# One-2-3-45/One-2-3-45

Hardware: NVIDIA H100
Metric: sec/mesh end-to-end (256x256 in) (lower is better)
Workload: dtype f16

## Files before the change

### one-2-3-45_b200/csrc/gemm_tc.cu

```cuda
#include <cuda.h>
#include <stdlib.h>
#include <cuda_fp16.h>

#include "common.cuh"
#include "wgmma.cuh"

namespace o2345 {
namespace {

constexpr int BM = 128, BK = 64;
constexpr int EPI_WARPS = 8;
constexpr int EPI_THREADS = 32 * EPI_WARPS;
constexpr int GEMM_THREADS = 128 + EPI_THREADS;
constexpr uint64_t WAIT_LIMIT_NS = 4000000000ull;
constexpr int MAX_CLUSTER = 8;
constexpr int RES_PREFETCH = 8;

enum { WAIT_EMPTY = 1, WAIT_FULL = 2 };

struct TrapRecord {
  unsigned long long magic;
  int tag, stage, bx, by, bz, rank, M, N, K, bn, mode, splits, conv;
};
constexpr unsigned long long TRAP_MAGIC = 0x6f32333435545250ull;

__device__ __forceinline__ uint32_t smem_u32(const void* p) { return (uint32_t)__cvta_generic_to_shared(p); }

__device__ __forceinline__ void mbar_init(uint64_t* bar, uint32_t count) {
  asm volatile("mbarrier.init.shared::cta.b64 [%0], %1;" ::"r"(smem_u32(bar)), "r"(count));
}
__device__ __forceinline__ void mbar_expect_tx(uint64_t* bar, uint32_t bytes) {
  asm volatile("mbarrier.arrive.expect_tx.shared::cta.b64 _, [%0], %1;" ::"r"(smem_u32(bar)), "r"(bytes) : "memory");
}
__device__ __forceinline__ void mbar_arrive(uint64_t* bar) {
  asm volatile("mbarrier.arrive.shared::cta.b64 _, [%0];" ::"r"(smem_u32(bar)) : "memory");
}
__device__ __forceinline__ uint32_t mbar_try(uint64_t* bar, uint32_t parity) {
  uint32_t done;
  asm volatile(
      "{\n\t.reg .pred p;\n\t"
      "mbarrier.try_wait.parity.shared::cta.b64 p, [%1], %2;\n\t"
      "selp.u32 %0, 1, 0, p;\n\t}"
      : "=r"(done)
      : "r"(smem_u32(bar)), "r"(parity)
      : "memory");
  return done;
}
__device__ __forceinline__ uint64_t global_ns() {
  uint64_t t;
  asm volatile("mov.u64 %0, %%globaltimer;" : "=l"(t));
  return t;
}
__device__ __forceinline__ void tma_load_2d(void* dst, const CUtensorMap* map, uint64_t* bar, int c0, int c1) {
  asm volatile(
      "cp.async.bulk.tensor.2d.shared::cluster.global.mbarrier::complete_tx::bytes [%0], [%1, {%3, %4}], [%2];"
      ::"r"(smem_u32(dst)), "l"(map), "r"(smem_u32(bar)), "r"(c0), "r"(c1)
      : "memory");
}
__device__ __forceinline__ void tma_load_4d(void* dst, const CUtensorMap* map, uint64_t* bar, int c0, int c1, int c2, int c3) {
  asm volatile(
      "cp.async.bulk.tensor.4d.shared::cluster.global.mbarrier::complete_tx::bytes [%0], [%1, {%3, %4, %5, %6}], [%2];"
      ::"r"(smem_u32(dst)), "l"(map), "r"(smem_u32(bar)), "r"(c0), "r"(c1), "r"(c2), "r"(c3)
      : "memory");
}
__device__ __forceinline__ uint32_t cluster_ctarank() {
  uint32_t r;
  asm volatile("mov.u32 %0, %%cluster_ctarank;" : "=r"(r));
  return r;
}
__device__ __forceinline__ void cluster_sync_all() {
  asm volatile("barrier.cluster.arrive.release.aligned;\n\tbarrier.cluster.wait.acquire.aligned;" ::: "memory");
}
__device__ __forceinline__ void epi_bar() { asm volatile("bar.sync 1, 256;" ::: "memory"); }

__host__ __device__ constexpr int acc_ld(int bn) { return bn + 4; }
__device__ __forceinline__ void acc_ld32(const float* src, uint32_t (&r)[32]) {
#pragma unroll
  for (int i = 0; i < 8; ++i) {
    const float4 v = reinterpret_cast<const float4*>(src)[i];
    r[4 * i] = __float_as_uint(v.x), r[4 * i + 1] = __float_as_uint(v.y), r[4 * i + 2] = __float_as_uint(v.z), r[4 * i + 3] = __float_as_uint(v.w);
  }
}

struct GemmParams {
  int M, N, K;
  int64_t ldc;
  int nh;
  int64_t stride_c_h, stride_c_b;
  const float* bias;
  const __half* rowbias;
  int64_t rowbias_ld;
  int rows_per_group;
  const __half* residual;
  void* C;
  int out_f32;
  int act;
// ... 211 lines not shown
  }
  const int share = (BM * BN + p.splits - 1) / p.splits;
  const int i1 = min(BM * BN, (z + 1) * share);
  for (int i = z * share + te; i < i1; i += EPI_THREADS) {
    const int rl = i / BN, row = m0 + rl, col = n0 + (i - rl * BN);
    if (row >= p.M || col >= p.N) continue;
    float x = 0.f;
    for (int s = 0; s < p.splits; ++s) x += __ldcg(p.ws + (int64_t)s * plane + (int64_t)row * p.N + col);
    x *= p.alpha;
    if (p.rowbias) x += __half2float(p.rowbias[(int64_t)(row / p.rows_per_group) * p.rowbias_ld + col]);
    if (p.bias) x += __ldg(p.bias + col);
    x = apply_act(x, p.act);
    const int64_t o = out_row(p, row) * p.ldc + col;
    if (p.residual) x += __half2float(p.residual[o]);
    if (p.out_f32) reinterpret_cast<float*>(p.C)[o] = x;
    else reinterpret_cast<__half*>(p.C)[o] = __float2half_rn(x);
  }
}

constexpr int EPI_RB_GROUPS = 8;
__host__ __device__ constexpr int epi_smem_bytes(int bn) { return bn * 4 + EPI_RB_GROUPS * bn * 2; }
__host__ __device__ constexpr int col_split(int bn) { return ((bn / 2 + 31) / 32) * 32; }

template <int BN>
__device__ __forceinline__ void epilogue_preload(const GemmParams& p, int m0, int n0, float* sbias, __half* srb, int te) {
  for (int i = te; i < BN; i += EPI_THREADS) sbias[i] = (p.bias && n0 + i < p.N) ? __ldg(p.bias + n0 + i) : 0.f;
  if (p.rowbias) {
    const int g0 = m0 / p.rows_per_group;
    const int last = (m0 + BM - 1 < p.M ? m0 + BM - 1 : p.M - 1) / p.rows_per_group;
    const int ng = last - g0 + 1;
    if (ng >= 1 && ng <= EPI_RB_GROUPS)
      for (int i = te; i < ng * BN; i += EPI_THREADS) {
        const int gi = i / BN, c = i - gi * BN;
        srb[i] = (n0 + c < p.N) ? p.rowbias[(int64_t)(g0 + gi) * p.rowbias_ld + n0 + c] : __float2half(0.f);
      }
  }
  epi_bar();
}

template <int ACT>
__device__ __forceinline__ float act_fn(float x) {
  if (ACT == 1) return __fdividef(x, 1.f + __expf(-x));
  if (ACT == 2) return gelu_erf(x);
  if (ACT == 4) return __fdividef(x, 1.f + __expf(-1.702f * x));
  return x;
}

template <int ACT>
__device__ __forceinline__ void stage_rows(const GemmParams& p, const float* acc_row, uint8_t* mine, int n0, int c_lo, int c_hi,
                                           const float* sbias, const __half* rb, bool rb_smem) {
#pragma unroll 1
  for (int c0 = c_lo; c0 < c_hi; c0 += 32) {
    if (n0 + c0 >= p.N) break;
    uint32_t r[32];
    acc_ld32(acc_row + c0, r);
    if (ACT == 3) {
      __half2 h[8];
#pragma unroll
      for (int e = 0; e < 16; e += 2) {
        float a0 = fmaf(__uint_as_float(r[e]), p.alpha, sbias[c0 + e]), a1 = fmaf(__uint_as_float(r[e + 1]), p.alpha, sbias[c0 + e + 1]);
        float g0 = fmaf(__uint_as_float(r[16 + e]), p.alpha, sbias[c0 + 16 + e]);
        float g1 = fmaf(__uint_as_float(r[17 + e]), p.alpha, sbias[c0 + 17 + e]);
        h[e >> 1] = __floats2half2_rn(a0 * gelu_erf_fast(g0), a1 * gelu_erf_fast(g1));
      }
      uint4* d = reinterpret_cast<uint4*>(mine + (c0 - c_lo));
      d[0] = reinterpret_cast<uint4*>(h)[0], d[1] = reinterpret_cast<uint4*>(h)[1];
    } else {
#pragma unroll
      for (int j = 0; j < 32; j += 8) {
        float v[8];
        const float4 b0 = *reinterpret_cast<const float4*>(sbias + c0 + j), b1 = *reinterpret_cast<const float4*>(sbias + c0 + j + 4);
        v[0] = b0.x, v[1] = b0.y, v[2] = b0.z, v[3] = b0.w, v[4] = b1.x, v[5] = b1.y, v[6] = b1.z, v[7] = b1.w;
        if (rb && (rb_smem || n0 + c0 + j + 8 <= p.N)) {
          uint4 q = *reinterpret_cast<const uint4*>(rb + c0 + j);
          const __half* hq = reinterpret_cast<const __half*>(&q);
#pragma unroll
          for (int e = 0; e < 8; ++e) v[e] += __half2float(hq[e]);
        }
        __half2 h[4];
#pragma unroll
        for (int e = 0; e < 8; e += 2) {
          float x0 = fmaf(__uint_as_float(r[j + e]), p.alpha, v[e]), x1 = fmaf(__uint_as_float(r[j + e + 1]), p.alpha, v[e + 1]);
          h[e >> 1] = __floats2half2_rn(act_fn<ACT>(x0), act_fn<ACT>(x1));
        }
        *reinterpret_cast<uint4*>(mine + (c0 - c_lo + j) * 2) = *reinterpret_cast<uint4*>(h);
      }
    }
  }
}

struct WarpOut {
  int outc, stride, ppr, total, ocol0, nout;
};
template <int MODE>
__device__ __forceinline__ WarpOut warp_out(const GemmParams& p, int n0, int c_lo, int c_hi) {
  constexpr bool geglu = MODE == 1;
  WarpOut g;
  g.outc = geglu ? (c_hi - c_lo) >> 1 : (c_hi - c_lo);
  g.stride = g.outc * 2 + 16;
  g.ppr = g.outc >> 3;
  g.total = 32 * g.ppr;
  g.ocol0 = geglu ? (n0 + c_lo) >> 1 : n0 + c_lo;
  g.nout = geglu ? p.N >> 1 : p.N;
  return g;
}

__device__ __forceinline__ void prefetch_residual(const GemmParams& p, const WarpOut& g, int lane, int row0,
                                                  uint4 (&resq)[RES_PREFETCH]) {
#pragma unroll
  for (int u = 0; u < RES_PREFETCH; ++u) {
    resq[u] = make_uint4(0u, 0u, 0u, 0u);
    const int pp = lane + 32 * u;
    if (p.residual && pp < g.total) {
      const int rl = pp / g.ppr, ci = pp - rl * g.ppr;
      const int grow = row0 + rl, col = g.ocol0 + ci * 8;
      if (grow < p.M && col < g.nout) resq[u] = *reinterpret_cast<const uint4*>(p.residual + out_row(p, grow) * p.ldc + col);
    }
  }
}

__device__ __forceinline__ uint4 add_h8(uint4 v, uint4 q) {
  __half2* a = reinterpret_cast<__half2*>(&v);
  const __half2* b = reinterpret_cast<const __half2*>(&q);
#pragma unroll
  for (int e = 0; e < 4; ++e) {
    float2 fa = __half22float2(a[e]), fb = __half22float2(b[e]);
    a[e] = __floats2half2_rn(fa.x + fb.x, fa.y + fb.y);
  }
  return v;
}

template <int BN, int MODE>
__device__ __forceinline__ void epilogue_staged(const GemmParams& p, const WarpOut& g, const float* acc_row, uint8_t* slab, int lane,
                                                int m0, int row0, int n0, int c_lo, int c_hi, const float* sbias, const __half* srb,
                                                const uint4 (&resq)[RES_PREFETCH]) {
  const int row = row0 + lane;
  const __half* rb = nullptr;
  bool rb_smem = false;
  if (MODE != 1 && p.rowbias) {
    const int rr = row < p.M ? row : p.M - 1;
    const int g0 = m0 / p.rows_per_group, last = (m0 + BM - 1 < p.M ? m0 + BM - 1 : p.M - 1) / p.rows_per_group;
    rb_smem = last - g0 + 1 <= EPI_RB_GROUPS;
    rb = rb_smem ? srb + (rr / p.rows_per_group - g0) * BN : p.rowbias + (int64_t)(rr / p.rows_per_group) * p.rowbias_ld + n0;
  }
  uint8_t* mine = slab + lane * g.stride;
  if (MODE == 0) {
    stage_rows<0>(p, acc_row, mine, n0, c_lo, c_hi, sbias, rb, rb_smem);
  } else if (MODE == 1) {
    stage_rows<3>(p, acc_row, mine, n0, c_lo, c_hi, sbias, rb, rb_smem);
  } else {
    switch (p.act) {
      case 1: stage_rows<1>(p, acc_row, mine, n0, c_lo, c_hi, sbias, rb, rb_smem); break;
      case 2: stage_rows<2>(p, acc_row, mine, n0, c_lo, c_hi, sbias, rb, rb_smem); break;
      default: stage_rows<4>(p, acc_row, mine, n0, c_lo, c_hi, sbias, rb, rb_smem); break;
    }
  }
  __syncwarp();
  __half* C = reinterpret_cast<__half*>(p.C);
#pragma unroll
  for (int u = 0; u < RES_PREFETCH; ++u) {
    const int pp = lane + 32 * u;
    if (pp < g.total) {
      const int rl = pp / g.ppr, ci = pp - rl * g.ppr;
      const int grow = row0 + rl, col = g.ocol0 + ci * 8;
      if (grow < p.M && col < g.nout) {
        uint4 v = *reinterpret_cast<const uint4*>(slab + rl * g.stride + ci * 16);
        if (p.residual) v = add_h8(v, resq[u]);
        *reinterpret_cast<uint4*>(C + out_row(p, grow) * p.ldc + col) = v;
      }
    }
  }
  constexpr int UN = 4;
  for (int base = lane + 32 * RES_PREFETCH; base < g.total; base += 32 * UN) {
    uint4 v[UN], q[UN];
    int64_t o[UN];
    bool ok[UN];
#pragma unroll
    for (int u = 0; u < UN; ++u) {
      const int pp = base + 32 * u;
      const int rl = pp / g.ppr, ci = pp - rl * g.ppr;
      const int grow = row0 + rl, col = g.ocol0 + ci * 8;
      ok[u] = pp < g.total && grow < p.M && col < g.nout;
      o[u] = out_row(p, grow) * p.ldc + col;
      if (ok[u]) {
        v[u] = *reinterpret_cast<const uint4*>(slab + rl * g.stride + ci * 16);
        if (p.residual) q[u] = *reinterpret_cast<const uint4*>(p.residual + o[u]);
      }
    }
#pragma unroll
    for (int u = 0; u < UN; ++u) {
      if (!ok[u]) continue;
      if (p.residual) v[u] = add_h8(v[u], q[u]);
      *reinterpret_cast<uint4*>(C + o[u]) = v[u];
    }
  }
}

__host__ __device__ constexpr int epi_slab_bytes(int bn) { return EPI_WARPS * 32 * (col_split(bn) * 2 + 16); }
constexpr int smem_bytes(int bn, int stages) {
  return stages * (BM * BK * 2 + bn * BK * 2) + epi_slab_bytes(bn) + 2 * stages * 8 + 16 + epi_smem_bytes(bn) + 1024;
}

struct ProducerPos {
  int x, y, b;
  int tap, tx, ty;
  int cb;
};
__device__ __forceinline__ ProducerPos producer_start(const GemmParams& p, int m0, int bz, int kb0) {
  ProducerPos q;
  q.x = q.y = q.b = q.tap = q.tx = q.ty = q.cb = 0;
  if (p.conv) {
    const int r = m0 / p.cW;
    q.x = m0 - r * p.cW, q.y = r % p.cH, q.b = r / p.cH;
    q.tap = kb0 / p.cblocks, q.cb = kb0 - q.tap * p.cblocks;
    q.ty = q.tap / p.ctx, q.tx = q.tap - q.ty * p.ctx;
  } else if (p.batched) {
    q.y = bz % p.nh, q.b = bz / p.nh;
  }
  return q;
}
__device__ __forceinline__ void producer_step(const GemmParams& p, ProducerPos& q) {
  if (p.conv && ++q.cb == p.cblocks) {
    q.cb = 0, ++q.tap;
// ... 10 lines not shown
    tma_load_4d(a_dst, tmA, full_bar, c0, q.x + q.tx + p.cox, q.y + q.ty + p.coy, q.b);
    tma_load_2d(b_dst, tmB, full_bar, q.tap * p.cC + c0, n0);
  } else if (p.batched) {
    tma_load_4d(a_dst, tmA, full_bar, kb * BK, m0, q.y, q.b);
    tma_load_4d(b_dst, tmB, full_bar, kb * BK, n0, q.y, q.b);
  } else {
    tma_load_2d(a_dst, tmA, full_bar, kb * BK, m0);
    tma_load_2d(b_dst, tmB, full_bar, kb * BK, n0);
  }
}

template <int BN>
__device__ __forceinline__ void acc_store(float* acc, const float (&d)[BN / 2], int row0, int t) {
  const int r = row0 + 16 * (t >> 5) + ((t & 31) >> 2), c = 2 * (t & 3);
#pragma unroll
  for (int j = 0; j < BN / 8; ++j) {
    *reinterpret_cast<float2*>(acc + r * acc_ld(BN) + 8 * j + c) = make_float2(d[4 * j], d[4 * j + 1]);
    *reinterpret_cast<float2*>(acc + (r + 8) * acc_ld(BN) + 8 * j + c) = make_float2(d[4 * j + 2], d[4 * j + 3]);
  }
}

template <int BN, int STAGES, int MODE>
__global__ void __launch_bounds__(GEMM_THREADS, 1)
gemm_tc_kernel(const __grid_constant__ CUtensorMap tmA, const __grid_constant__ CUtensorMap tmB, const __grid_constant__ GemmParams p) {
  extern __shared__ __align__(1024) uint8_t smem_raw[];
  uint8_t* smem = reinterpret_cast<uint8_t*>((reinterpret_cast<uintptr_t>(smem_raw) + 1023) & ~(uintptr_t)1023);
  constexpr int A_BYTES = BM * BK * 2, B_BYTES = BN * BK * 2;
  static_assert(B_BYTES % 1024 == 0, "stage bases must stay 1024-byte aligned for SWIZZLE_128B");
  static_assert(BN % 32 == 0 && BN >= 64 && BN <= 256, "tile width: a multiple of 32 (GEGLU chunks, 32-column epilogue reads)");
  static_assert(BM * acc_ld(BN) * 4 <= STAGES * (A_BYTES + B_BYTES), "the accumulator tile must fit in the operand ring");
  constexpr int CSPLIT = col_split(BN);
  uint8_t* sA = smem;
  uint8_t* sB = smem + STAGES * A_BYTES;
  uint8_t* slabs = sB + STAGES * B_BYTES;
  uint64_t* full = reinterpret_cast<uint64_t*>(slabs + epi_slab_bytes(BN));
  uint64_t* empty = full + STAGES;
  float* sbias = reinterpret_cast<float*>((reinterpret_cast<uintptr_t>(empty + STAGES) + 15) & ~(uintptr_t)15);
  __half* srb = reinterpret_cast<__half*>(sbias + BN);
  float* acc = reinterpret_cast<float*>(smem);

  const int warp = threadIdx.x >> 5, lane = threadIdx.x & 31;
  if (threadIdx.x == 0) stamp(p, 0), stamp_ns(p, 16);
  const int bz = blockIdx.z;
  const int nk = p.conv ? p.ctaps * p.cblocks : (p.K + BK - 1) / BK;
  const bool split = MODE == 3 && p.splits > 1;
  int kb0 = 0, kb1 = nk;
  if (split) {
    kb0 = (int)((int64_t)nk * bz / p.splits);
    kb1 = (int)((int64_t)nk * (bz + 1) / p.splits);
  }

  if (threadIdx.x == 0) {
    asm volatile("prefetch.tensormap [%0];" ::"l"(&tmA) : "memory");
    asm volatile("prefetch.tensormap [%0];" ::"l"(&tmB) : "memory");
    for (int s = 0; s < STAGES; ++s) mbar_init(full + s, 1), mbar_init(empty + s, 2);
    asm volatile("fence.mbarrier_init.release.cluster;" ::: "memory");
    asm volatile("fence.proxy.async.shared::cta;" ::: "memory");
  }
  __syncthreads();
  pdl_wait();
  pdl_trigger();
  if (threadIdx.x == 0) stamp(p, 1);

  const int tiles_m = (p.M + BM - 1) / BM, tiles = tiles_m * ((p.N + BN - 1) / BN);
  const bool persist = MODE != 3 && p.persist;
  uint32_t cnt = 0;
  for (int t = persist ? blockIdx.x : blockIdx.y * tiles_m + blockIdx.x; t < tiles; t += persist ? gridDim.x : tiles) {
  const int m0 = (t % tiles_m) * BM, n0 = (t / tiles_m) * BN;
  if (warp < 4) {
    if (threadIdx.x == 0) {
      asm volatile("fence.proxy.async.shared::cta;" ::: "memory");
      ProducerPos q = producer_start(p, m0, bz, kb0);
      for (int kb = kb0; kb < kb1; ++kb) {
        const uint32_t c = cnt + (kb - kb0);
        const int s = c % STAGES;
        const uint32_t ph = (c / STAGES) & 1;
        mbar_wait(empty + s, ph ^ 1, p, WAIT_EMPTY, s);
        produce_stage<BN>(p, &tmA, &tmB, sA + s * A_BYTES, sB + s * B_BYTES, full + s, kb, m0, n0, q);
        producer_step(p, q);
        if (kb == kb0) stamp(p, 2);
      }
      stamp(p, 3);
    }
    __syncwarp();
  } else {
    const int wg = (warp >> 2) - 1, e = warp - 4, quarter = e & 3, te = threadIdx.x - 128;
    const int c_lo = e < 4 ? 0 : CSPLIT, c_hi = e < 4 ? CSPLIT : BN;
    const int row0 = m0 + quarter * 32;
    if (MODE != 3) epilogue_preload<BN>(p, m0, n0, sbias, srb, te);
    {
      float d[BN / 2];
#pragma unroll
      for (int i = 0; i < BN / 2; ++i) d[i] = 0.f;
      for (int kb = kb0; kb < kb1; ++kb) {
        const uint32_t c = cnt + (kb - kb0);
        const int s = c % STAGES;
        const uint32_t ph = (c / STAGES) & 1;
        mbar_wait(full + s, ph, p, WAIT_FULL, s);
        if (kb == kb0 && te == 0) stamp(p, 4);
        const uint32_t a0 = smem_u32(sA + s * A_BYTES) + wg * (64 * 128), b0 = smem_u32(sB + s * B_BYTES);
        wg::fence();
#pragma unroll
        for (int k = 0; k < BK / 16; ++k)
          wg::mma_f16<BN>(d, wg::desc_sw128(a0 + k * 32), wg::desc_sw128(b0 + k * 32), 1);
        wg::commit();
        wg::wait<1>();
        if (kb > kb0 && (threadIdx.x & 127) == 0) mbar_arrive(empty + (c - 1) % STAGES);
      }
      wg::wait<0>();
      if ((threadIdx.x & 127) == 0) mbar_arrive(empty + (cnt + kb1 - kb0 - 1) % STAGES);
      if (te == 0) stamp(p, 5);
      epi_bar();
      acc_store<BN>(acc, d, 64 * wg, threadIdx.x & 127);
    }
    epi_bar();
    if (te == 0) stamp(p, 6);
    const float* acc_row = acc + (quarter * 32 + lane) * acc_ld(BN);
    if (MODE != 3) {
      const WarpOut g = warp_out<MODE>(p, n0, c_lo, c_hi);
      uint4 resq[RES_PREFETCH];
      prefetch_residual(p, g, lane, row0, resq);
      epilogue_staged<BN, MODE>(p, g, acc_row, slabs + e * 32 * (CSPLIT * 2 + 16), lane, m0, row0, n0, c_lo, c_hi, sbias, srb, resq);
    } else {
      const int row = row0 + lane;
      if (split) {
        if (te == 0) stamp_ns(p, 17);
#pragma unroll 1
        for (int c0 = c_lo; c0 < c_hi; c0 += 32) {
          uint32_t r[32];
          acc_ld32(acc_row + c0, r);
          if (row < p.M) splitk_partial(p, r, bz, row, n0 + c0);
        }
        if (te == 0) stamp_ns(p, 18);
      } else {
        const int64_t crow = (p.batched ? (int64_t)(bz % p.nh) * p.stride_c_h + (int64_t)(bz / p.nh) * p.stride_c_b : 0) +
                             out_row(p, row < p.M ? row : 0) * p.ldc;
#pragma unroll 1
        for (int c0 = c_lo; c0 < c_hi; c0 += 32) {
          uint32_t r[32];
          acc_ld32(acc_row + c0, r);
          if (row < p.M) epilogue_chunk(p, r, row, crow, n0 + c0);
        }
      }
    }
    if (te == 0) stamp(p, 7);
  }
  cnt += kb1 - kb0;
  __syncthreads();
  }
  if (split) {
    cluster_sync_all();
    if (warp >= 4) {
      if (threadIdx.x == 128) stamp_ns(p, 21, true);
      splitk_finalize<BN>(p, blockIdx.x * BM, blockIdx.y * BN, bz, threadIdx.x - 128);
      if (threadIdx.x == 128) stamp_ns(p, 22, true);
    }
  }
  if (threadIdx.x == 0) stamp(p, 8);
}

typedef CUresult (*EncodeTiledFn)(CUtensorMap*, CUtensorMapDataType, cuuint32_t, void*, const cuuint64_t*, const cuuint64_t*,
                                  const cuuint32_t*, const cuuint32_t*, CUtensorMapInterleave, CUtensorMapSwizzle,
                                  CUtensorMapL2promotion, CUtensorMapFloatOOBfill);

EncodeTiledFn encode_fn() {
  static EncodeTiledFn fn = nullptr;
  if (!fn) {
    void* p = nullptr;
    cudaDriverEntryPointQueryResult q;
    if (cudaGetDriverEntryPoint("cuTensorMapEncodeTiled", &p, cudaEnableDefault, &q) == cudaSuccess && q == cudaDriverEntryPointSuccess)
      fn = reinterpret_cast<EncodeTiledFn>(p);
  }
  return fn;
}

int make_map(CUtensorMap* m, const void* ptr, int64_t rows, int64_t K, int64_t ld, int nh, int nb, int64_t sh, int64_t sb,
             int box_rows) {
  EncodeTiledFn fn = encode_fn();
  if (!fn) { set_error("cuTensorMapEncodeTiled entry point not available"); return O2345_ECUDA; }
  cuuint64_t dims[4] = {(cuuint64_t)K, (cuuint64_t)rows, (cuuint64_t)(nh > 0 ? nh : 1), (cuuint64_t)(nb > 0 ? nb : 1)};
  cuuint64_t strides[3] = {(cuuint64_t)ld * 2, (cuuint64_t)sh * 2, (cuuint64_t)sb * 2};
  cuuint32_t box[4] = {(cuuint32_t)BK, (cuuint32_t)box_rows, 1, 1};
  cuuint32_t estr[4] = {1, 1, 1, 1};
  int rank = nh > 0 ? 4 : 2;
  CUresult r = fn(m, CU_TENSOR_MAP_DATA_TYPE_FLOAT16, rank, const_cast<void*>(ptr), dims, strides, box, estr,
                  CU_TENSOR_MAP_INTERLEAVE_NONE, CU_TENSOR_MAP_SWIZZLE_128B, CU_TENSOR_MAP_L2_PROMOTION_L2_256B,
                  CU_TENSOR_MAP_FLOAT_OOB_FILL_NONE);
  if (r != CUDA_SUCCESS) { set_error("cuTensorMapEncodeTiled failed with %d (rows=%lld K=%lld ld=%lld)", (int)r, (long long)rows, (long long)K, (long long)ld); return O2345_ECUDA; }
  return O2345_OK;
}

TrapRecord* g_diag = nullptr;
bool g_diag_tried = false;
TrapRecord* diag_buffer(cudaStream_t st) {
  if (!g_diag_tried) {
    cudaStreamCaptureStatus cs = cudaStreamCaptureStatusNone;
    if (cudaStreamIsCapturing(st, &cs) != cudaSuccess || cs != cudaStreamCaptureStatusNone) {
      cudaGetLastError();
      return g_diag;
    }
    g_diag_tried = true;
    void* h = nullptr;
    if (cudaHostAlloc(&h, sizeof(TrapRecord), cudaHostAllocMapped | cudaHostAllocPortable) == cudaSuccess) {
      memset(h, 0, sizeof(TrapRecord));
      g_diag = reinterpret_cast<TrapRecord*>(h);
    } else {
      cudaGetLastError();
    }
  }
  return g_diag;
}
// ... 47 lines not shown
  static const int kBn[4] = {64, 128, 160, 256};
  static const int kSplits[6] = {1, 2, 3, 4, 6, 8};
  const bool split_ok = can_split && p.act != 3 && p.ws && 2 * (int64_t)M * N <= ws_floats;
  const int max_planes = split_ok ? (int)(ws_floats / ((int64_t)M * N)) : 1;
  float best = 1e30f;
  c.bn = 128, c.splits = 1;
  for (int bi = 0; bi < 4; ++bi) {
    const int bn = kBn[bi];
    if (bn > 64 && N <= 64) continue;
    if (g_force[1] > 0 && bn != g_force[1]) continue;
    for (int si = 0; si < 6; ++si) {
      const int sp = kSplits[si];
      if (g_force[2] > 0 && sp != (g_force[2] > nk ? nk : g_force[2])) continue;
      if (sp > 1 && (!split_ok || sp > max_planes || sp > MAX_CLUSTER || nk / sp < 3)) continue;
      const float us = predict_us(M, N, nk, bn, sp);
      if (us < best) best = us, c.bn = bn, c.splits = sp;
    }
  }
  if (best > 1e29f) {
    c.bn = (g_force[1] == 64 || g_force[1] == 128 || g_force[1] == 160 || g_force[1] == 256) ? g_force[1] : 128;
    c.splits = 1;
  }
  const int tiles = cdiv(M, BM) * cdiv(N, c.bn);
  const int min_tiles = g_persist_min_tiles > 0 ? g_persist_min_tiles : 4 * sm_count();
  c.persist = c.splits == 1 && (g_persist == 1 || (g_persist == 0 && tiles >= min_tiles));
  return c;
}

int pick_mode(const GemmParams& p, const Config& c) {
  const int nout = p.act == 3 ? p.N / 2 : p.N;
  const bool staged = !p.out_f32 && c.splits <= 1 && !p.batched && (nout % 8) == 0 && (p.ldc % 8) == 0 && ((uintptr_t)p.C % 16) == 0 &&
                      (!p.residual || ((uintptr_t)p.residual % 16) == 0);
  if (!staged) return 3;
  return p.act == 0 ? 0 : (p.act == 3 ? 1 : 2);
}

long long* g_trace = nullptr;

template <int BN, int STAGES, int MODE>
int launch(const CUtensorMap& a, const CUtensorMap& b, GemmParams p, int batch, int persist, cudaStream_t st) {
  constexpr int SMEM = smem_bytes(BN, STAGES);
  static_assert(SMEM <= 227 * 1024, "one CTA per SM");
  static PerDeviceOnce attr;
  if (attr.need())
    O2345_CUDA(cudaFuncSetAttribute(gemm_tc_kernel<BN, STAGES, MODE>, cudaFuncAttributeMaxDynamicSharedMemorySize, SMEM));
  p.bn = BN, p.mode = MODE;
  p.diag = diag_buffer(st);
  const int splits = (MODE == 3 && batch == 0 && p.splits > 1) ? p.splits : 1;
  p.splits = splits;
  dim3 grid(cdiv(p.M, BM), cdiv(p.N, BN), batch > 0 ? batch : splits);
  p.persist = MODE != 3 && batch == 0 && splits == 1 && persist;
  if (p.persist) {
    const int tiles = (int)grid.x * (int)grid.y;
    grid = dim3(tiles < sm_count() ? tiles : sm_count(), 1, 1);
  }
  O2345_CUDA(launch_pdl_cluster(gemm_tc_kernel<BN, STAGES, MODE>, grid, dim3(GEMM_THREADS), (size_t)SMEM, st, 1, splits, a, b, p));
  O2345_LAUNCH_CHECK();
  return O2345_OK;
}

template <int BN, int STAGES>
int launch_mode(int mode, const CUtensorMap& a, const CUtensorMap& b, const GemmParams& p, int batch, int persist, cudaStream_t st) {
  switch (mode) {
    case 0: return launch<BN, STAGES, 0>(a, b, p, batch, persist, st);
    case 1: return launch<BN, STAGES, 1>(a, b, p, batch, persist, st);
    case 2: return launch<BN, STAGES, 2>(a, b, p, batch, persist, st);
    default: return launch<BN, STAGES, 3>(a, b, p, batch, persist, st);
  }
}

int dispatch(const Config& c, int mode, const CUtensorMap& a, const CUtensorMap& b, const GemmParams& p, int batch, cudaStream_t st) {
  if (c.bn == 64) return launch_mode<64, 6>(mode, a, b, p, batch, c.persist, st);
  if (c.bn == 128) return launch_mode<128, 5>(mode, a, b, p, batch, c.persist, st);
  if (c.bn == 160) return launch_mode<160, 4>(mode, a, b, p, batch, c.persist, st);
  return launch_mode<256, 3>(mode, a, b, p, batch, c.persist, st);
}

int fill_epilogue(GemmParams& p, const o2345_epilogue* ep, int N, int64_t ldc) {
  p.bias = nullptr, p.rowbias = nullptr, p.rowbias_ld = 0, p.rows_per_group = 1, p.residual = nullptr;
// ... 18 lines not shown

using namespace o2345;

extern "C" void o2345_debug_gemm_trace(long long* device_buf16) { g_trace = device_buf16; }

extern "C" void o2345_debug_gemm_force(int ctas, int bn, int splits) {
  read_force_env();
  g_force[0] = ctas, g_force[1] = bn, g_force[2] = splits;
}


extern "C" void o2345_debug_gemm_persist(int mode, int min_tiles) { g_persist = mode, g_persist_min_tiles = min_tiles; }

extern "C" void o2345_debug_gemm_model(const float* seven) {
  for (int i = 0; i < 7; ++i) g_model[i] = seven[i];
}

extern "C" int o2345_last_trap(char* buf, size_t n) {
  if (!buf || n == 0) return O2345_EINVAL;
  buf[0] = 0;
  const TrapRecord* d = g_diag;
  if (!d || d->magic != TRAP_MAGIC) return 0;
  static const char* names[] = {"?", "empty (producer waiting for the MMA to free a stage)", "full (MMA issuer waiting for TMA bytes)",
                                };
  snprintf(buf, n,
           "gemm_tc_kernel<BN=%d, MODE=%d> M=%d N=%d K=%d conv=%d splits=%d: CTA (%d,%d,%d) rank %d gave up after 4 s "
           "on barrier '%s' stage %d",
           d->bn, d->mode, d->M, d->N, d->K, d->conv, d->splits, d->bx, d->by, d->bz, d->rank,
           names[d->tag >= 1 && d->tag <= 2 ? d->tag : 0], d->stage);
  return 1;
}

namespace o2345 {
namespace {
int conv_launch(const void* x, int B, int H, int W, int C, const void* weight, int N, void* out, int64_t ldc, const o2345_epilogue* ep,
                float* splitk_ws, int64_t ws_floats, int taps, int tx, int ox, int oy, int up, int upa, int upb, cudaStream_t st) {
  EncodeTiledFn fn = encode_fn();
  if (!fn) { set_error("cuTensorMapEncodeTiled entry point not available"); return O2345_ECUDA; }
  const int tw = W >= 128 ? 128 : W;
  const int th = W >= 128 ? 1 : (128 / W < H ? 128 / W : H);
  const int tb = 128 / (tw * th);
  CUtensorMap ma, mb;
  {
    cuuint64_t dims[4] = {(cuuint64_t)C, (cuuint64_t)W, (cuuint64_t)H, (cuuint64_t)B};
    cuuint64_t strides[3] = {(cuuint64_t)C * 2, (cuuint64_t)W * C * 2, (cuuint64_t)H * W * C * 2};
    cuuint32_t box[4] = {(cuuint32_t)BK, (cuuint32_t)tw, (cuuint32_t)th, (cuuint32_t)tb};
    cuuint32_t estr[4] = {1, 1, 1, 1};
    CUresult r = fn(&ma, CU_TENSOR_MAP_DATA_TYPE_FLOAT16, 4, const_cast<void*>(x), dims, strides, box, estr,
                    CU_TENSOR_MAP_INTERLEAVE_NONE, CU_TENSOR_MAP_SWIZZLE_128B, CU_TENSOR_MAP_L2_PROMOTION_L2_256B,
                    CU_TENSOR_MAP_FLOAT_OOB_FILL_NONE);
    if (r != CUDA_SUCCESS) { set_error("cuTensorMapEncodeTiled (conv activation) failed with %d", (int)r); return O2345_ECUDA; }
  }
// ... 80 lines not shown
```

Baseline: 2.483.

## Write GEMM epilogue from registers via swizzled smem and TMA stores

Replaces the accumulator-to-smem round trip and per-warp staged global stores with a per-warpgroup epilogue that converts the MMA registers directly into a swizzled shared-memory output tile. The tile goes to global memory with TMA bulk tensor stores, and the residual is brought in by a TMA load that is issued early and overlaps the main loop. Bias and rowbias preload moves into each warpgroup and overlaps the first MMA; it also lowers the persistent-kernel tile threshold. This aims to cut epilogue shared-memory traffic and uncoalesced stores, and to overlap the epilogue with the next tile. It adds host tensor-map encoding on every launch and constraints on output layouts.

```diff
diff --git a/one-2-3-45_b200/csrc/gemm_tc.cu b/one-2-3-45_b200/csrc/gemm_tc.cu
--- a/one-2-3-45_b200/csrc/gemm_tc.cu
+++ b/one-2-3-45_b200/csrc/gemm_tc.cu
@@ -14,9 +14,8 @@
 constexpr int GEMM_THREADS = 128 + EPI_THREADS;
 constexpr uint64_t WAIT_LIMIT_NS = 4000000000ull;
 constexpr int MAX_CLUSTER = 8;
-constexpr int RES_PREFETCH = 8;
-
-enum { WAIT_EMPTY = 1, WAIT_FULL = 2 };
+
+enum { WAIT_EMPTY = 1, WAIT_FULL = 2, WAIT_RESIDUAL = 3 };
 
 struct TrapRecord {
   unsigned long long magic;
@@ -63,6 +62,18 @@
       ::"r"(smem_u32(dst)), "l"(map), "r"(smem_u32(bar)), "r"(c0), "r"(c1), "r"(c2), "r"(c3)
       : "memory");
 }
+__device__ __forceinline__ void tma_store_2d(const CUtensorMap* map, const void* src, int c0, int c1) {
+  asm volatile("cp.async.bulk.tensor.2d.global.shared::cta.bulk_group [%0, {%2, %3}], [%1];"
+               ::"l"(map), "r"(smem_u32(src)), "r"(c0), "r"(c1) : "memory");
+}
+__device__ __forceinline__ void tma_store_5d(const CUtensorMap* map, const void* src, int c0, int c1, int c2, int c3, int c4) {
+  asm volatile("cp.async.bulk.tensor.5d.global.shared::cta.bulk_group [%0, {%2, %3, %4, %5, %6}], [%1];"
+               ::"l"(map), "r"(smem_u32(src)), "r"(c0), "r"(c1), "r"(c2), "r"(c3), "r"(c4) : "memory");
+}
+__device__ __forceinline__ void bulk_commit() { asm volatile("cp.async.bulk.commit_group;" ::: "memory"); }
+__device__ __forceinline__ void bulk_wait_read() { asm volatile("cp.async.bulk.wait_group.read 0;" ::: "memory"); }
+__device__ __forceinline__ void bulk_wait() { asm volatile("cp.async.bulk.wait_group 0;" ::: "memory"); }
+__device__ __forceinline__ void fence_proxy_async() { asm volatile("fence.proxy.async.shared::cta;" ::: "memory"); }
 __device__ __forceinline__ uint32_t cluster_ctarank() {
   uint32_t r;
   asm volatile("mov.u32 %0, %%cluster_ctarank;" : "=r"(r));
@@ -72,6 +83,7 @@
   asm volatile("barrier.cluster.arrive.release.aligned;\n\tbarrier.cluster.wait.acquire.aligned;" ::: "memory");
 }
 __device__ __forceinline__ void epi_bar() { asm volatile("bar.sync 1, 256;" ::: "memory"); }
+__device__ __forceinline__ void wg_bar(int wg) { asm volatile("bar.sync %0, 128;" ::"r"(2 + wg) : "memory"); }
 
 __host__ __device__ constexpr int acc_ld(int bn) { return bn + 4; }
 __device__ __forceinline__ void acc_ld32(const float* src, uint32_t (&r)[32]) {
@@ -329,20 +341,37 @@
 __host__ __device__ constexpr int epi_smem_bytes(int bn) { return bn * 4 + EPI_RB_GROUPS * bn * 2; }
 __host__ __device__ constexpr int col_split(int bn) { return ((bn / 2 + 31) / 32) * 32; }
 
+__host__ __device__ constexpr int out_cols(int bn, int mode) { return mode == 1 ? bn / 2 : bn; }
+__host__ __device__ constexpr int out_box(int ow) { return ow % 64 == 0 ? 64 : (ow % 32 == 0 ? 32 : 16); }
+__host__ __device__ constexpr int out_half_bytes(int ow) { return 64 * ow * 2; }
+
+template <int BOX>
+__device__ __forceinline__ uint32_t out_off(int r, int c) {
+  const uint32_t o = (uint32_t)(r * (2 * BOX) + (c % BOX) * 2);
+  return (uint32_t)(c / BOX) * (128 * BOX) + (o ^ (((o >> 7) & (BOX / 8 - 1)) << 4));
+}
+__device__ __forceinline__ uint32_t ld_shared_u32(uint32_t a) {
+  uint32_t v;
+  asm volatile("ld.shared.b32 %0, [%1];" : "=r"(v) : "r"(a) : "memory");
+  return v;
+}
+__device__ __forceinline__ void st_shared_u32(uint32_t a, uint32_t v) { asm volatile("st.shared.b32 [%0], %1;" ::"r"(a), "r"(v) : "memory"); }
+__device__ __forceinline__ uint32_t h2_bits(__half2 h) { return *reinterpret_cast<uint32_t*>(&h); }
+__device__ __forceinline__ __half2 bits_h2(uint32_t v) { return *reinterpret_cast<__half2*>(&v); }
+
 template <int BN>
-__device__ __forceinline__ void epilogue_preload(const GemmParams& p, int m0, int n0, float* sbias, __half* srb, int te) {
-  for (int i = te; i < BN; i += EPI_THREADS) sbias[i] = (p.bias && n0 + i < p.N) ? __ldg(p.bias + n0 + i) : 0.f;
-  if (p.rowbias) {
-    const int g0 = m0 / p.rows_per_group;
-    const int last = (m0 + BM - 1 < p.M ? m0 + BM - 1 : p.M - 1) / p.rows_per_group;
+__device__ __forceinline__ void epilogue_preload(const GemmParams& p, int rm0, int n0, float* sbias, __half* srb, int tw) {
+  for (int i = tw; i < BN; i += 128) sbias[i] = (p.bias && n0 + i < p.N) ? __ldg(p.bias + n0 + i) : 0.f;
+  if (p.rowbias && rm0 < p.M) {
+    const int g0 = rm0 / p.rows_per_group;
+    const int last = (rm0 + 63 < p.M ? rm0 + 63 : p.M - 1) / p.rows_per_group;
     const int ng = last - g0 + 1;
-    if (ng >= 1 && ng <= EPI_RB_GROUPS)
-      for (int i = te; i < ng * BN; i += EPI_THREADS) {
+    if (ng <= EPI_RB_GROUPS)
+      for (int i = tw; i < ng * BN; i += 128) {
         const int gi = i / BN, c = i - gi * BN;
         srb[i] = (n0 + c < p.N) ? p.rowbias[(int64_t)(g0 + gi) * p.rowbias_ld + n0 + c] : __float2half(0.f);
       }
   }
-  epi_bar();
 }
 
 template <int ACT>
@@ -353,159 +382,70 @@
   return x;
 }
 
-template <int ACT>
-__device__ __forceinline__ void stage_rows(const GemmParams& p, const float* acc_row, uint8_t* mine, int n0, int c_lo, int c_hi,
-                                           const float* sbias, const __half* rb, bool rb_smem) {
-#pragma unroll 1
-  for (int c0 = c_lo; c0 < c_hi; c0 += 32) {
-    if (n0 + c0 >= p.N) break;
-    uint32_t r[32];
-    acc_ld32(acc_row + c0, r);
-    if (ACT == 3) {
-      __half2 h[8];
-#pragma unroll
-      for (int e = 0; e < 16; e += 2) {
-        float a0 = fmaf(__uint_as_float(r[e]), p.alpha, sbias[c0 + e]), a1 = fmaf(__uint_as_float(r[e + 1]), p.alpha, sbias[c0 + e + 1]);
-        float g0 = fmaf(__uint_as_float(r[16 + e]), p.alpha, sbias[c0 + 16 + e]);
-        float g1 = fmaf(__uint_as_float(r[17 + e]), p.alpha, sbias[c0 + 17 + e]);
-        h[e >> 1] = __floats2half2_rn(a0 * gelu_erf_fast(g0), a1 * gelu_erf_fast(g1));
-      }
-      uint4* d = reinterpret_cast<uint4*>(mine + (c0 - c_lo));
-      d[0] = reinterpret_cast<uint4*>(h)[0], d[1] = reinterpret_cast<uint4*>(h)[1];
-    } else {
-#pragma unroll
-      for (int j = 0; j < 32; j += 8) {
-        float v[8];
-        const float4 b0 = *reinterpret_cast<const float4*>(sbias + c0 + j), b1 = *reinterpret_cast<const float4*>(sbias + c0 + j + 4);
-        v[0] = b0.x, v[1] = b0.y, v[2] = b0.z, v[3] = b0.w, v[4] = b1.x, v[5] = b1.y, v[6] = b1.z, v[7] = b1.w;
-        if (rb && (rb_smem || n0 + c0 + j + 8 <= p.N)) {
-          uint4 q = *reinterpret_cast<const uint4*>(rb + c0 + j);
-          const __half* hq = reinterpret_cast<const __half*>(&q);
-#pragma unroll
-          for (int e = 0; e < 8; ++e) v[e] += __half2float(hq[e]);
+template <int BN, int MODE, int ACT>
+__device__ __forceinline__ void epilogue_regs(const GemmParams& p, const float (&d)[BN / 2], uint32_t tile, int tw, int n0,
+                                              const float* sbias, const __half* const (&rb)[2], bool rb_global) {
+  constexpr int BOX = out_box(out_cols(BN, MODE));
+  const int q = tw & 3, r = 16 * (tw >> 5) + ((tw & 31) >> 2);
+  if constexpr (MODE == 1) {
+#pragma unroll
+    for (int k = 0; k < BN / 32; ++k)
+#pragma unroll
+      for (int jj = 0; jj < 2; ++jj) {
+        const int j = 4 * k + jj, c = 8 * j + 2 * q;
+        const float2 bv = *reinterpret_cast<const float2*>(sbias + c), bg = *reinterpret_cast<const float2*>(sbias + c + 16);
+#pragma unroll
+        for (int h = 0; h < 2; ++h) {
+          const float a0 = fmaf(d[4 * j + 2 * h], p.alpha, bv.x), a1 = fmaf(d[4 * j + 2 * h + 1], p.alpha, bv.y);
+          const float g0 = fmaf(d[4 * (j + 2) + 2 * h], p.alpha, bg.x), g1 = fmaf(d[4 * (j + 2) + 2 * h + 1], p.alpha, bg.y);
+          st_shared_u32(tile + out_off<BOX>(r + 8 * h, 16 * k + 8 * jj + 2 * q),
+                        h2_bits(__floats2half2_rn(a0 * gelu_erf_fast(g0), a1 * gelu_erf_fast(g1))));
         }
-        __half2 h[4];
-#pragma unroll
-        for (int e = 0; e < 8; e += 2) {
-          float x0 = fmaf(__uint_as_float(r[j + e]), p.alpha, v[e]), x1 = fmaf(__uint_as_float(r[j + e + 1]), p.alpha, v[e + 1]);
-          h[e >> 1] = __floats2half2_rn(act_fn<ACT>(x0), act_fn<ACT>(x1));
-        }
-        *reinterpret_cast<uint4*>(mine + (c0 - c_lo + j) * 2) = *reinterpret_cast<uint4*>(h);
-      }
-    }
-  }
-}
-
-struct WarpOut {
-  int outc, stride, ppr, total, ocol0, nout;
-};
-template <int MODE>
-__device__ __forceinline__ WarpOut warp_out(const GemmParams& p, int n0, int c_lo, int c_hi) {
-  constexpr bool geglu = MODE == 1;
-  WarpOut g;
-  g.outc = geglu ? (c_hi - c_lo) >> 1 : (c_hi - c_lo);
-  g.stride = g.outc * 2 + 16;
-  g.ppr = g.outc >> 3;
-  g.total = 32 * g.ppr;
-  g.ocol0 = geglu ? (n0 + c_lo) >> 1 : n0 + c_lo;
-  g.nout = geglu ? p.N >> 1 : p.N;
-  return g;
-}
-
-__device__ __forceinline__ void prefetch_residual(const GemmParams& p, const WarpOut& g, int lane, int row0,
-                                                  uint4 (&resq)[RES_PREFETCH]) {
-#pragma unroll
-  for (int u = 0; u < RES_PREFETCH; ++u) {
-    resq[u] = make_uint4(0u, 0u, 0u, 0u);
-    const int pp = lane + 32 * u;
-    if (p.residual && pp < g.total) {
-      const int rl = pp / g.ppr, ci = pp - rl * g.ppr;
-      const int grow = row0 + rl, col = g.ocol0 + ci * 8;
-      if (grow < p.M && col < g.nout) resq[u] = *reinterpret_cast<const uint4*>(p.residual + out_row(p, grow) * p.ldc + col);
-    }
-  }
-}
-
-__device__ __forceinline__ uint4 add_h8(uint4 v, uint4 q) {
-  __half2* a = reinterpret_cast<__half2*>(&v);
-  const __half2* b = reinterpret_cast<const __half2*>(&q);
-#pragma unroll
-  for (int e = 0; e < 4; ++e) {
-    float2 fa = __half22float2(a[e]), fb = __half22float2(b[e]);
-    a[e] = __floats2half2_rn(fa.x + fb.x, fa.y + fb.y);
-  }
-  return v;
-}
-
-template <int BN, int MODE>
-__device__ __forceinline__ void epilogue_staged(const GemmParams& p, const WarpOut& g, const float* acc_row, uint8_t* slab, int lane,
-                                                int m0, int row0, int n0, int c_lo, int c_hi, const float* sbias, const __half* srb,
-                                                const uint4 (&resq)[RES_PREFETCH]) {
-  const int row = row0 + lane;
-  const __half* rb = nullptr;
-  bool rb_smem = false;
-  if (MODE != 1 && p.rowbias) {
-    const int rr = row < p.M ? row : p.M - 1;
-    const int g0 = m0 / p.rows_per_group, last = (m0 + BM - 1 < p.M ? m0 + BM - 1 : p.M - 1) / p.rows_per_group;
-    rb_smem = last - g0 + 1 <= EPI_RB_GROUPS;
-    rb = rb_smem ? srb + (rr / p.rows_per_group - g0) * BN : p.rowbias + (int64_t)(rr / p.rows_per_group) * p.rowbias_ld + n0;
-  }
-  uint8_t* mine = slab + lane * g.stride;
-  if (MODE == 0) {
-    stage_rows<0>(p, acc_row, mine, n0, c_lo, c_hi, sbias, rb, rb_smem);
-  } else if (MODE == 1) {
-    stage_rows<3>(p, acc_row, mine, n0, c_lo, c_hi, sbias, rb, rb_smem);
+      }
   } else {
-    switch (p.act) {
-      case 1: stage_rows<1>(p, acc_row, mine, n0, c_lo, c_hi, sbias, rb, rb_smem); break;
-      case 2: stage_rows<2>(p, acc_row, mine, n0, c_lo, c_hi, sbias, rb, rb_smem); break;
-      default: stage_rows<4>(p, acc_row, mine, n0, c_lo, c_hi, sbias, rb, rb_smem); break;
-    }
-  }
-  __syncwarp();
-  __half* C = reinterpret_cast<__half*>(p.C);
-#pragma unroll
-  for (int u = 0; u < RES_PREFETCH; ++u) {
-    const int pp = lane + 32 * u;
-    if (pp < g.total) {
-      const int rl = pp / g.ppr, ci = pp - rl * g.ppr;
-      const int grow = row0 + rl, col = g.ocol0 + ci * 8;
-      if (grow < p.M && col < g.nout) {
-        uint4 v = *reinterpret_cast<const uint4*>(slab + rl * g.stride + ci * 16);
-        if (p.residual) v = add_h8(v, resq[u]);
-        *reinterpret_cast<uint4*>(C + out_row(p, grow) * p.ldc + col) = v;
-      }
-    }
-  }
-  constexpr int UN = 4;
-  for (int base = lane + 32 * RES_PREFETCH; base < g.total; base += 32 * UN) {
-    uint4 v[UN], q[UN];
-    int64_t o[UN];
-    bool ok[UN];
-#pragma unroll
-    for (int u = 0; u < UN; ++u) {
-      const int pp = base + 32 * u;
-      const int rl = pp / g.ppr, ci = pp - rl * g.ppr;
-      const int grow = row0 + rl, col = g.ocol0 + ci * 8;
-      ok[u] = pp < g.total && grow < p.M && col < g.nout;
-      o[u] = out_row(p, grow) * p.ldc + col;
-      if (ok[u]) {
-        v[u] = *reinterpret_cast<const uint4*>(slab + rl * g.stride + ci * 16);
-        if (p.residual) q[u] = *reinterpret_cast<const uint4*>(p.residual + o[u]);
-      }
-    }
-#pragma unroll
-    for (int u = 0; u < UN; ++u) {
-      if (!ok[u]) continue;
-      if (p.residual) v[u] = add_h8(v[u], q[u]);
-      *reinterpret_cast<uint4*>(C + o[u]) = v[u];
-    }
-  }
-}
-
-__host__ __device__ constexpr int epi_slab_bytes(int bn) { return EPI_WARPS * 32 * (col_split(bn) * 2 + 16); }
-constexpr int smem_bytes(int bn, int stages) {
-  return stages * (BM * BK * 2 + bn * BK * 2) + epi_slab_bytes(bn) + 2 * stages * 8 + 16 + epi_smem_bytes(bn) + 1024;
+#pragma unroll
+  for (int j = 0; j < BN / 8; ++j) {
+    const int c = 8 * j + 2 * q;
+    const float2 b = *reinterpret_cast<const float2*>(sbias + c);
+#pragma unroll
+    for (int h = 0; h < 2; ++h) {
+      float v0 = b.x, v1 = b.y;
+      if (rb[h] && (!rb_global || n0 + c < p.N)) {
+        const float2 f = __half22float2(*reinterpret_cast<const __half2*>(rb[h] + c));
+        v0 += f.x, v1 += f.y;
+      }
+      const float x0 = fmaf(d[4 * j + 2 * h], p.alpha, v0), x1 = fmaf(d[4 * j + 2 * h + 1], p.alpha, v1);
+      __half2 o = __floats2half2_rn(act_fn<ACT>(x0), act_fn<ACT>(x1));
+      const uint32_t a = tile + out_off<BOX>(r + 8 * h, c);
+      if (p.residual) {
+        const float2 fa = __half22float2(o), fb = __half22float2(bits_h2(ld_shared_u32(a)));
+        o = __floats2half2_rn(fa.x + fb.x, fa.y + fb.y);
+      }
+      st_shared_u32(a, h2_bits(o));
+    }
+  }
+  }
+}
+
+template <int BOX, int NBOX, bool STORE>
+__device__ __forceinline__ void out_tile_tma(const GemmParams& p, const CUtensorMap* map, uint8_t* tile, int rm0, int ocol0, int nout,
+                                             uint64_t* bar) {
+  const int nb = min(NBOX, (nout - ocol0 + BOX - 1) / BOX);
+  if (!STORE) mbar_expect_tx(bar, (uint32_t)nb * (128 * BOX));
+#pragma unroll
+  for (int b = 0; b < NBOX; ++b) {
+    if (b >= nb) break;
+    const int c = ocol0 + b * BOX;
+    uint8_t* s = tile + b * (128 * BOX);
+    if (!STORE) tma_load_2d(s, map, bar, c, rm0);
+    else if (p.up) tma_store_5d(map, s, c, p.upb, rm0 % p.cW, p.upa, rm0 / p.cW);
+    else tma_store_2d(map, s, c, rm0);
+  }
+}
+
+constexpr int smem_bytes(int bn, int stages, int mode) {
+  return stages * (BM * BK * 2 + bn * BK * 2) + (mode == 3 ? 0 : 2 * out_half_bytes(out_cols(bn, mode))) + (2 * stages + 2) * 8 + 16 +
+         2 * epi_smem_bytes(bn) + 1024;
 }
 
 struct ProducerPos {
@@ -562,7 +502,8 @@
 
 template <int BN, int STAGES, int MODE>
 __global__ void __launch_bounds__(GEMM_THREADS, 1)
-gemm_tc_kernel(const __grid_constant__ CUtensorMap tmA, const __grid_constant__ CUtensorMap tmB, const __grid_constant__ GemmParams p) {
+gemm_tc_kernel(const __grid_constant__ CUtensorMap tmA, const __grid_constant__ CUtensorMap tmB, const __grid_constant__ CUtensorMap tmC,
+               const __grid_constant__ CUtensorMap tmR, const __grid_constant__ GemmParams p) {
   extern __shared__ __align__(1024) uint8_t smem_raw[];
   uint8_t* smem = reinterpret_cast<uint8_t*>((reinterpret_cast<uintptr_t>(smem_raw) + 1023) & ~(uintptr_t)1023);
   constexpr int A_BYTES = BM * BK * 2, B_BYTES = BN * BK * 2;
@@ -570,13 +511,15 @@
   static_assert(BN % 32 == 0 && BN >= 64 && BN <= 256, "tile width: a multiple of 32 (GEGLU chunks, 32-column epilogue reads)");
   static_assert(BM * acc_ld(BN) * 4 <= STAGES * (A_BYTES + B_BYTES), "the accumulator tile must fit in the operand ring");
   constexpr int CSPLIT = col_split(BN);
+  constexpr int OW = out_cols(BN, MODE), BOX = out_box(OW), OUT_HALF = out_half_bytes(OW);
   uint8_t* sA = smem;
   uint8_t* sB = smem + STAGES * A_BYTES;
-  uint8_t* slabs = sB + STAGES * B_BYTES;
-  uint64_t* full = reinterpret_cast<uint64_t*>(slabs + epi_slab_bytes(BN));
+  uint8_t* sOut = sB + STAGES * B_BYTES;
+  uint64_t* full = reinterpret_cast<uint64_t*>(sOut + (MODE == 3 ? 0 : 2 * OUT_HALF));
   uint64_t* empty = full + STAGES;
-  float* sbias = reinterpret_cast<float*>((reinterpret_cast<uintptr_t>(empty + STAGES) + 15) & ~(uintptr_t)15);
-  __half* srb = reinterpret_cast<__half*>(sbias + BN);
+  uint64_t* resbar = empty + STAGES;
+  float* sbias = reinterpret_cast<float*>((reinterpret_cast<uintptr_t>(resbar + 2) + 15) & ~(uintptr_t)15);
+  __half* srb = reinterpret_cast<__half*>(sbias + 2 * BN);
   float* acc = reinterpret_cast<float*>(smem);
 
   const int warp = threadIdx.x >> 5, lane = threadIdx.x & 31;
@@ -593,9 +536,11 @@
   if (threadIdx.x == 0) {
     asm volatile("prefetch.tensormap [%0];" ::"l"(&tmA) : "memory");
     asm volatile("prefetch.tensormap [%0];" ::"l"(&tmB) : "memory");
+    if (MODE != 3) asm volatile("prefetch.tensormap [%0];" ::"l"(&tmC) : "memory");
     for (int s = 0; s < STAGES; ++s) mbar_init(full + s, 1), mbar_init(empty + s, 2);
+    mbar_init(resbar, 1), mbar_init(resbar + 1, 1);
     asm volatile("fence.mbarrier_init.release.cluster;" ::: "memory");
-    asm volatile("fence.proxy.async.shared::cta;" ::: "memory");
+    fence_proxy_async();
   }
   __syncthreads();
   pdl_wait();
@@ -605,11 +550,11 @@
   const int tiles_m = (p.M + BM - 1) / BM, tiles = tiles_m * ((p.N + BN - 1) / BN);
   const bool persist = MODE != 3 && p.persist;
   uint32_t cnt = 0;
+  uint32_t rphase = 0;
   for (int t = persist ? blockIdx.x : blockIdx.y * tiles_m + blockIdx.x; t < tiles; t += persist ? gridDim.x : tiles) {
   const int m0 = (t % tiles_m) * BM, n0 = (t / tiles_m) * BN;
   if (warp < 4) {
     if (threadIdx.x == 0) {
-      asm volatile("fence.proxy.async.shared::cta;" ::: "memory");
       ProducerPos q = producer_start(p, m0, bz, kb0);
       for (int kb = kb0; kb < kb1; ++kb) {
         const uint32_t c = cnt + (kb - kb0);
@@ -624,10 +569,12 @@
     }
     __syncwarp();
   } else {
-    const int wg = (warp >> 2) - 1, e = warp - 4, quarter = e & 3, te = threadIdx.x - 128;
-    const int c_lo = e < 4 ? 0 : CSPLIT, c_hi = e < 4 ? CSPLIT : BN;
-    const int row0 = m0 + quarter * 32;
-    if (MODE != 3) epilogue_preload<BN>(p, m0, n0, sbias, srb, te);
+    const int wg = (warp >> 2) - 1, e = warp - 4, quarter = e & 3, te = threadIdx.x - 128, tw = threadIdx.x & 127;
+    const int rm0 = m0 + 64 * wg, ocol0 = MODE == 1 ? n0 / 2 : n0, nout = MODE == 1 ? p.N / 2 : p.N;
+    const bool rows = rm0 < p.M;
+    uint8_t* tile = sOut + wg * OUT_HALF;
+    float* wbias = sbias + wg * BN;
+    __half* wrb = srb + wg * EPI_RB_GROUPS * BN;
     {
       float d[BN / 2];
 #pragma unroll
@@ -637,32 +584,76 @@
         const int s = c % STAGES;
         const uint32_t ph = (c / STAGES) & 1;
         mbar_wait(full + s, ph, p, WAIT_FULL, s);
-        if (kb == kb0 && te == 0) stamp(p, 4);
+        if (kb == kb0 && te == 0) {
+          if (p.trace && t != (int)blockIdx.x && blockIdx.x == 0 && blockIdx.y == 0 && blockIdx.z == 0) p.trace[9] = p.trace[5];
+          stamp(p, 4);
+        }
         const uint32_t a0 = smem_u32(sA + s * A_BYTES) + wg * (64 * 128), b0 = smem_u32(sB + s * B_BYTES);
         wg::fence();
 #pragma unroll
         for (int k = 0; k < BK / 16; ++k)
           wg::mma_f16<BN>(d, wg::desc_sw128(a0 + k * 32), wg::desc_sw128(b0 + k * 32), 1);
         wg::commit();
+        if (MODE != 3 && kb == kb0) {
+          if (tw == 0) {
+            bulk_wait_read();
+            if (p.residual && rows) out_tile_tma<BOX, OW / BOX, false>(p, &tmR, tile, rm0, ocol0, nout, resbar + wg);
+          }
+          epilogue_preload<BN>(p, rm0, n0, wbias, wrb, tw);
+          wg_bar(wg);
+        }
         wg::wait<1>();
-        if (kb > kb0 && (threadIdx.x & 127) == 0) mbar_arrive(empty + (c - 1) % STAGES);
+        if (kb > kb0 && tw == 0) mbar_arrive(empty + (c - 1) % STAGES);
       }
       wg::wait<0>();
-      if ((threadIdx.x & 127) == 0) mbar_arrive(empty + (cnt + kb1 - kb0 - 1) % STAGES);
+      if (tw == 0) mbar_arrive(empty + (cnt + kb1 - kb0 - 1) % STAGES);
       if (te == 0) stamp(p, 5);
+      if (MODE != 3) {
+        if (rows) {
+          if (p.residual) mbar_wait(resbar + wg, rphase & 1, p, WAIT_RESIDUAL, wg);
+          if (te == 0) stamp(p, 6);
+          const __half* rb[2] = {nullptr, nullptr};
+          bool rb_global = false;
+          if (MODE != 1 && p.rowbias) {
+            const int g0 = rm0 / p.rows_per_group, last = (rm0 + 63 < p.M ? rm0 + 63 : p.M - 1) / p.rows_per_group;
+            rb_global = last - g0 + 1 > EPI_RB_GROUPS;
+#pragma unroll
+            for (int h = 0; h < 2; ++h) {
+              const int row = rm0 + 16 * (tw >> 5) + ((tw & 31) >> 2) + 8 * h, g = (row < p.M ? row : p.M - 1) / p.rows_per_group;
+              rb[h] = rb_global ? p.rowbias + (int64_t)g * p.rowbias_ld + n0 : wrb + (g - g0) * BN;
+            }
+          }
+          const uint32_t ts = smem_u32(tile);
+          if constexpr (MODE == 0) {
+            epilogue_regs<BN, 0, 0>(p, d, ts, tw, n0, wbias, rb, rb_global);
+          } else if constexpr (MODE == 1) {
+            epilogue_regs<BN, 1, 3>(p, d, ts, tw, n0, wbias, rb, rb_global);
+          } else {
+            switch (p.act) {
+              case 1: epilogue_regs<BN, 2, 1>(p, d, ts, tw, n0, wbias, rb, rb_global); break;
+              case 2: epilogue_regs<BN, 2, 2>(p, d, ts, tw, n0, wbias, rb, rb_global); break;
+              default: epilogue_regs<BN, 2, 4>(p, d, ts, tw, n0, wbias, rb, rb_global); break;
+            }
+          }
+          fence_proxy_async();
+          wg_bar(wg);
+          if (tw == 0) {
+            out_tile_tma<BOX, OW / BOX, true>(p, &tmC, tile, rm0, ocol0, nout, nullptr);
+            bulk_commit();
+          }
+          if (p.residual) ++rphase;
+        }
+      } else {
+        epi_bar();
+        acc_store<BN>(acc, d, 64 * wg, tw);
+      }
+    }
+    if (MODE == 3) {
       epi_bar();
-      acc_store<BN>(acc, d, 64 * wg, threadIdx.x & 127);
-    }
-    epi_bar();
-    if (te == 0) stamp(p, 6);
-    const float* acc_row = acc + (quarter * 32 + lane) * acc_ld(BN);
-    if (MODE != 3) {
-      const WarpOut g = warp_out<MODE>(p, n0, c_lo, c_hi);
-      uint4 resq[RES_PREFETCH];
-      prefetch_residual(p, g, lane, row0, resq);
-      epilogue_staged<BN, MODE>(p, g, acc_row, slabs + e * 32 * (CSPLIT * 2 + 16), lane, m0, row0, n0, c_lo, c_hi, sbias, srb, resq);
-    } else {
-      const int row = row0 + lane;
+      if (te == 0) stamp(p, 6);
+      const float* acc_row = acc + (quarter * 32 + lane) * acc_ld(BN);
+      const int c_lo = e < 4 ? 0 : CSPLIT, c_hi = e < 4 ? CSPLIT : BN;
+      const int row = m0 + quarter * 32 + lane;
       if (split) {
         if (te == 0) stamp_ns(p, 17);
 #pragma unroll 1
@@ -686,8 +677,9 @@
     if (te == 0) stamp(p, 7);
   }
   cnt += kb1 - kb0;
-  __syncthreads();
-  }
+  if (MODE == 3) __syncthreads();
+  }
+  if (MODE != 3 && warp >= 4 && (threadIdx.x & 127) == 0) bulk_wait();
   if (split) {
     cluster_sync_all();
     if (warp >= 4) {
@@ -727,6 +719,32 @@
                   CU_TENSOR_MAP_INTERLEAVE_NONE, CU_TENSOR_MAP_SWIZZLE_128B, CU_TENSOR_MAP_L2_PROMOTION_L2_256B,
                   CU_TENSOR_MAP_FLOAT_OOB_FILL_NONE);
   if (r != CUDA_SUCCESS) { set_error("cuTensorMapEncodeTiled failed with %d (rows=%lld K=%lld ld=%lld)", (int)r, (long long)rows, (long long)K, (long long)ld); return O2345_ECUDA; }
+  return O2345_OK;
+}
+
+int make_out_map(CUtensorMap* m, const void* ptr, const GemmParams& p, int nout, int box) {
+  EncodeTiledFn fn = encode_fn();
+  if (!fn) { set_error("cuTensorMapEncodeTiled entry point not available"); return O2345_ECUDA; }
+  const CUtensorMapSwizzle sw = box == 64 ? CU_TENSOR_MAP_SWIZZLE_128B : (box == 32 ? CU_TENSOR_MAP_SWIZZLE_64B : CU_TENSOR_MAP_SWIZZLE_32B);
+  const cuuint64_t row = (cuuint64_t)p.ldc * 2;
+  cuuint32_t estr[5] = {1, 1, 1, 1, 1};
+  CUresult r;
+  if (p.up) {
+    O2345_CHECK_ARG(64 % p.cW == 0 || p.cW % 64 == 0, "up-sampling conv output map: W must divide 64 or be a multiple of 64");
+    const int wt = p.cW < 64 ? p.cW : 64;
+    cuuint64_t dims[5] = {(cuuint64_t)nout, 2, (cuuint64_t)p.cW, 2, (cuuint64_t)(p.M / p.cW)};
+    cuuint64_t strides[4] = {row, 2 * row, 2 * (cuuint64_t)p.cW * row, 4 * (cuuint64_t)p.cW * row};
+    cuuint32_t boxd[5] = {(cuuint32_t)box, 1, (cuuint32_t)wt, 1, (cuuint32_t)(64 / wt)};
+    r = fn(m, CU_TENSOR_MAP_DATA_TYPE_FLOAT16, 5, const_cast<void*>(ptr), dims, strides, boxd, estr, CU_TENSOR_MAP_INTERLEAVE_NONE, sw,
+           CU_TENSOR_MAP_L2_PROMOTION_L2_256B, CU_TENSOR_MAP_FLOAT_OOB_FILL_NONE);
+  } else {
+    cuuint64_t dims[2] = {(cuuint64_t)nout, (cuuint64_t)p.M};
+    cuuint64_t strides[1] = {row};
+    cuuint32_t boxd[2] = {(cuuint32_t)box, 64};
+    r = fn(m, CU_TENSOR_MAP_DATA_TYPE_FLOAT16, 2, const_cast<void*>(ptr), dims, strides, boxd, estr, CU_TENSOR_MAP_INTERLEAVE_NONE, sw,
+           CU_TENSOR_MAP_L2_PROMOTION_L2_256B, CU_TENSOR_MAP_FLOAT_OOB_FILL_NONE);
+  }
+  if (r != CUDA_SUCCESS) { set_error("cuTensorMapEncodeTiled (GEMM output) failed with %d (M=%d nout=%d ldc=%lld)", (int)r, p.M, nout, (long long)p.ldc); return O2345_ECUDA; }
   return O2345_OK;
 }
 
@@ -820,7 +838,7 @@
     c.splits = 1;
   }
   const int tiles = cdiv(M, BM) * cdiv(N, c.bn);
-  const int min_tiles = g_persist_min_tiles > 0 ? g_persist_min_tiles : 4 * sm_count();
+  const int min_tiles = g_persist_min_tiles > 0 ? g_persist_min_tiles : 2 * sm_count();
   c.persist = c.splits == 1 && (g_persist == 1 || (g_persist == 0 && tiles >= min_tiles));
   return c;
 }
@@ -837,7 +855,7 @@
 
 template <int BN, int STAGES, int MODE>
 int launch(const CUtensorMap& a, const CUtensorMap& b, GemmParams p, int batch, int persist, cudaStream_t st) {
-  constexpr int SMEM = smem_bytes(BN, STAGES);
+  constexpr int SMEM = smem_bytes(BN, STAGES, MODE);
   static_assert(SMEM <= 227 * 1024, "one CTA per SM");
   static PerDeviceOnce attr;
   if (attr.need())
@@ -852,7 +870,14 @@
     const int tiles = (int)grid.x * (int)grid.y;
     grid = dim3(tiles < sm_count() ? tiles : sm_count(), 1, 1);
   }
-  O2345_CUDA(launch_pdl_cluster(gemm_tc_kernel<BN, STAGES, MODE>, grid, dim3(GEMM_THREADS), (size_t)SMEM, st, 1, splits, a, b, p));
+  CUtensorMap mc, mr;
+  memset(&mc, 0, sizeof(mc)), memset(&mr, 0, sizeof(mr));
+  if (MODE != 3) {
+    constexpr int OW = out_cols(BN, MODE);
+    O2345_TRY(make_out_map(&mc, p.C, p, p.act == 3 ? p.N / 2 : p.N, out_box(OW)));
+    if (p.residual) O2345_TRY(make_out_map(&mr, p.residual, p, p.N, out_box(OW)));
+  }
+  O2345_CUDA(launch_pdl_cluster(gemm_tc_kernel<BN, STAGES, MODE>, grid, dim3(GEMM_THREADS), (size_t)SMEM, st, 1, splits, a, b, mc, mr, p));
   O2345_LAUNCH_CHECK();
   return O2345_OK;
 }
@@ -917,12 +942,12 @@
   const TrapRecord* d = g_diag;
   if (!d || d->magic != TRAP_MAGIC) return 0;
   static const char* names[] = {"?", "empty (producer waiting for the MMA to free a stage)", "full (MMA issuer waiting for TMA bytes)",
-                                };
+                                "residual (epilogue waiting for the TMA load of its residual half tile)"};
   snprintf(buf, n,
            "gemm_tc_kernel<BN=%d, MODE=%d> M=%d N=%d K=%d conv=%d splits=%d: CTA (%d,%d,%d) rank %d gave up after 4 s "
            "on barrier '%s' stage %d",
            d->bn, d->mode, d->M, d->N, d->K, d->conv, d->splits, d->bx, d->by, d->bz, d->rank,
-           names[d->tag >= 1 && d->tag <= 2 ? d->tag : 0], d->stage);
+           names[d->tag >= 1 && d->tag <= 3 ? d->tag : 0], d->stage);
   return 1;
 }
 
```

Measured after the change: 2.372 (median of 6 runs). -4.5%, faster.
